# Alan-404/Conformer

Measured on AMD Instinct MI355X. Metric: encoder audio-frames/sec (B=32,T=1000,d=512,L=16), higher is better.
Workload: dtype f32

## Files before the change

### conformer_amd/_lib.py

```python
from __future__ import annotations

import ctypes
import os
from ctypes import c_char_p, c_float, c_int, c_int64, c_uint64, c_void_p

_HERE = os.path.dirname(os.path.abspath(__file__))
LIB_PATH = os.environ.get("CONFORMER_AMD_LIB") or os.path.join(_HERE, "lib", "libconformer_hip.so")

_P, _I, _L, _F, _U = c_void_p, c_int, c_int64, c_float, c_uint64
ABI_VERSION = 4

SIGNATURES = {
    "cfm_version": (c_int, []),
    "cfm_abi_version": (c_int, []),
    "cfm_gemm_bias_stats_f32": (c_int, [_P, _P, _P, _P, _P, _L, _I, _I, _L, _L, _P]),
    "cfm_gemm_bias_residual_stats_f32": (c_int, [_P, _P, _P, _P, _F, _P, _P, _L, _I, _I, _L, _L, _L, _P]),
    "cfm_gemm_splitk_f32": (c_int, [_I, _P, _P, _P, _P, _F, _P, _P, _I, _L, _I, _I, _L, _L, _L, _P]),
    "cfm_gemm_lnfold_f32": (c_int, [_I, _P, _P, _I, _F, _P, _P, _P, _P, _L, _I, _I, _L, _L, _P]),
    "cfm_layernorm_fwd_stats_f32": (c_int, [_P, _P, _P, _P, _P, _L, _I, _F, _P]),
    "cfm_ffn_pack_elems": (ctypes.c_int64, [_I, _I]),
    "cfm_ffn_pack_f32": (c_int, [_P, _P, _P, _I, _I, _P]),
    "cfm_rowgemm_pack_f32": (c_int, [_P, _P, _I, _I, _I, _P]),
    "cfm_rowchain_f32": (c_int, [_I, _I, _I, _I, _P, _L, _P, _P, _P, _L, _P, _L, _P, _I, _F, _P, _P, _P, _P, _F, _I, _P, _L, _P, _P, _P, _F,
                                 _P, _P, _P, _F, _P, _L, _L, _I, _P]),
# ... 33 lines not shown
    "cfm_subsample_conv1_bwd_d16_f32": (c_int, [_I, _P, _P, _P, _P, _P, _P, _I, _I, _I, _I, _P]),
    "cfm_reflect_pad_f32": (c_int, [_P, _P, _I, _L, _I, _L, _P]),
    "cfm_power_mel_log_f32": (c_int, [_P, _L, _P, _P, _I, _I, _I, _I, _F, _P]),
    "cfm_power_mel_log_mfma_f32": (c_int, [_P, _L, _P, _P, _I, _I, _I, _I, _I, _F, _P]),
    "cfm_dft_frames_f32": (c_int, [_P, _P, _P, _L, _I, _I, _I, _P]),
    "cfm_specaugment_apply_f32": (c_int, [_P, _I, _I, _I, _P, _I, _F, _P]),
    "cfm_gemm_bias_swish_save_f32": (c_int, [_P, _P, _P, _P, _P, _L, _I, _I, _L, _L, _P]),
    "cfm_gemm_bwd_f32": (c_int, [_P, _I, _L, _P, _I, _L, _P, _L, _F, _P, _L, _I, _I, _L, _I, _P]),
    "cfm_gemm_bwd_batched_f32": (c_int, [_P, _I, _L, _P, _I, _L, _P, _L, _F, _P, _L, _I, _I, _L, _I, _I, _I, _I,
                                         _L, _L, _L, _L, _L, _L, _F, _U, _P]),
    "cfm_gemm_train_f32": (c_int, [_I, _P, _P, _P, _P, _F, _P, _P, _L, _I, _I, _L, _L, _L, _F, _U, _P]),
    "cfm_relpos_attention_train_f32": (c_int, [_P, _P, _P, _L, _P, _L, _P, _P, _P, _P, _L, _P, _I, _I, _I, _I, _F, _U, _P]),
    "cfm_dropout_f32": (c_int, [_P, _P, _L, _F, _U, _P]),
    "cfm_dropout_out16_f32": (c_int, [_I, _P, _P, _L, _F, _U, _P]),
    "cfm_layernorm_bwd_dx_f32": (c_int, [_P, _P, _P, _P, _P, _P, _P, _L, _I, _P]),
    "cfm_layernorm_bwd_params_f32": (c_int, [_P, _P, _P, _P, _P, _P, _L, _I, _P]),
    "cfm_layernorm_bwd_f32": (c_int, [_P, _P, _P, _P, _P, _P, _P, _P, _P, _L, _I, _P, ctypes.c_size_t, _P]),
    "cfm_layernorm_bwd_workspace_bytes": (ctypes.c_size_t, [_L, _I]),
    "cfm_colsum_f32": (c_int, [_P, _L, _L, _I, _F, _P, _P]),
    "cfm_glu_fwd_f32": (c_int, [_P, _P, _L, _I, _P]),
    "cfm_glu_bwd_f32": (c_int, [_P, _P, _P, _L, _I, _P]),
    "cfm_dwconv_bn_swish_bwd_f32": (c_int, [_P, _P, _P, _P, _P, _P, _P, _P, _F, _I, _P, _P, _P, _P, _P, _P,
                                            _I, _I, _I, _I, _P]),
    "cfm_dwconv_bn_stats_workspace_bytes": (ctypes.c_size_t, [_I, _I, _I]),
    "cfm_dwconv_bn_stats_f32": (c_int, [_P, _P, _P, _P, _P, _P, _P, _F, _I, _I, _I, _I, _P, ctypes.c_size_t, _P]),
    "cfm_debug_attention_bwd_trace_f32": (c_int, [_P]),
    "cfm_debug_attention_bwd_trace_mfma16": (c_int, [_P]),
    "cfm_debug_gemm_mfma16_trace": (c_int, [_P]),
    "cfm_debug_gemm_mfma16_force_tile": (c_int, [_I]),
    "cfm_relpos_attention_bwd_mfma16_f32": (c_int, [_I, _P, _P, _P, _L, _P, _L, _P, _P, _P, _P, _P, _L, _P, _P, _P, _P, _L, _P, _L,
                                                    _P, _P, _I, _I, _I, _I, _F, _U, _P]),
    "cfm_relpos_attention_bwd_f32": (c_int, [_P, _P, _P, _L, _P, _L, _P, _P, _P, _P, _P, _L, _P, _P, _P, _P, _L, _P, _L, _P, _P,
                                             _I, _I, _I, _I, _F, _U, _I, _P]),
    "cfm_relu_bwd_f32": (c_int, [_P, _P, _P, _L, _P]),
    "cfm_subsample_conv2_bwd_weight_f32": (c_int, [_P, _P, _P, _I, _I, _I, _I, _P]),
    "cfm_pack_conv2_weight_t_f32": (c_int, [_P, _P, _I, _P]),
    "cfm_subsample_conv2_bwd_input_f32": (c_int, [_P, _P, _P, _I, _I, _I, _I, _P]),
    "cfm_subsample_conv1_bwd_f32": (c_int, [_P, _P, _P, _P, _P, _P, _I, _I, _I, _I, _P]),
    "cfm_adam_step_f32": (c_int, [_P, _I, _F, _F, _F, _F, _F, _F, _P]),
    "cfm_greedy_ctc_decode_f32": (c_int, [_P, _P, _P, _P, _P, _I, _I, _I, _I, _I, _P]),
    "cfm_ctc_beam_workspace_bytes": (ctypes.c_size_t, [_I, _I, _I, _I]),
    "cfm_ctc_beam_decode_f32": (c_int, [_P, _P, _I, _I, _I, _I, _I, _I, _F, _F, _I, _P, ctypes.c_size_t, _P, _P, _P, _P, _P]),
    "cfm_ngram_lm_pack_bytes": (ctypes.c_size_t, [_I, _P, _I, _L, _I, _L]),
    "cfm_ngram_lm_pack": (c_int, [_I, _P, _P, _P, _P, _I, _P, _P, _I, _I, _I, _I, _P, _P, _P, _P, ctypes.c_size_t]),
    "cfm_ngram_lm_score_f64": (c_int, [_P, _P, _P, _I, _I, _P, _P]),
    "cfm_ctc_beam_lm_workspace_bytes": (ctypes.c_size_t, [_I, _I, _I, _I]),
    "cfm_ctc_beam_lm_decode_f32": (c_int, [_P, _P, _I, _I, _I, _I, _I, _I, _F, _F, _I, _P, ctypes.c_double, ctypes.c_double,
                                           ctypes.c_double, _I, _P, ctypes.c_size_t, _P, _P, _P, _P, _P, _P]),
    "cfm_lstm_fwd_f32": (c_int, [_P, _P, _P, _P, _P, _P, _P, _I, _I, _I, _P]),
    "cfm_lstm_fwd_frag_f32": (c_int, [_P, _P, _P, _P, _P, _P, _P, _P, _I, _I, _I, _P]),
    "cfm_lstm_bwd_frag_f32": (c_int, [_P, _P, _P, _P, _P, _P, _P, _P, _I, _I, _I, _P]),
    "cfm_debug_lstm_trace": (c_int, [_P]),
    "cfm_debug_dw16_trace": (c_int, [_P]),
    "cfm_linear_bwd_weight_mfma16_f32": (c_int, [_I, _P, _I, _L, _P, _I, _L, _P, _L, _P, _I, _I, _L, _F, _P]),
    "cfm_lstm_fwd_mfma16_f32": (c_int, [_I, _P, _P, _P, _P, _P, _P, _P, _P, _I, _I, _I, _P]),
    "cfm_lstm_bwd_mfma16_f32": (c_int, [_I, _P, _P, _P, _P, _P, _P, _P, _P, _I, _I, _I, _P]),
    "cfm_lstm_bwd_f32": (c_int, [_P, _P, _P, _P, _P, _P, _P, _I, _I, _I, _P]),
    "cfm_swish_bn_eval_f32": (c_int, [_P, _P, _P, _P, _P, _F, _P, _L, _I, _P]),
    "cfm_swish_bn_stats_f32": (c_int, [_P, _P, _P, _P, _P, _F, _L, _I, _P]),
    "cfm_swish_bn_bwd_f32": (c_int, [_P, _P, _P, _P, _P, _F, _I, _P, _P, _P, _L, _I, _P]),
    "cfm_split_pack_elems": (ctypes.c_int64, [_I, _I, _I]),
    "cfm_split_pack_bf16_f32": (c_int, [_I, _P, _P, _I, _I, _P]),
    "cfm_gemm_split_bf16_f32": (c_int, [_I, _I, _P, _P, _P, _P, _F, _P, _L, _I, _I, _L, _L, _L, _P]),
    "cfm_subsample_conv2_relu_split_bf16_f32": (c_int, [_I, _P, _P, _P, _P, _I, _I, _I, _I, _P]),
    "cfm_ctc_workspace_floats": (ctypes.c_int64, [_I, _I, _I]),
    "cfm_ctc_loss_fwd_f32": (c_int, [_P, _P, _P, _L, _L, _P, _P, _I, _I, _I, _I, _I, _P, _P, _P]),
    "cfm_ctc_loss_bwd_f32": (c_int, [_P, _P, _P, _L, _L, _P, _P, _I, _I, _I, _I, _I, _P, _P, _P, _P]),
    "cfm_relpos_attention_rows_f32": (c_int, [_P, _P, _P, _L, _P, _L, _P, _P, _P, _P, _L, _I, _I, _I, _I, _I, _I, _I, _P, _P]),
    "cfm_debug_attention_trace_f32": (c_int, [_P, _P, _P, _L, _P, _L, _P, _P, _P, _P, _L, _I, _I, _I, _I, _P, _P]),
    "cfm_debug_set_bwd_tile": (c_int, [_I]),
    "cfm_debug_set_attention_waves": (c_int, [_I]),
    "cfm_debug_gemm_cfg_f32": (c_int, [_I, _P, _P, _P, _P, _F, _P, _L, _I, _I, _P, _P]),
    "cfm_debug_set_conv2_bk": (c_int, [_I]),
    "cfm_debug_ffn_trace": (c_int, [_P, _I]),
    "cfm_debug_ffn_variant": (c_int, [_I]),
    "cfm_debug_ffn_layout": (c_int, [_I, _I]),
    "cfm_relpos_table_f32": (c_int, [_P, _P, _I, _I, _P]),
    "cfm_relpos_attention_fwd_f32": (c_int, [_P, _P, _P, _L, _P, _L, _P, _P, _P, _P, _L, _P, _I, _I, _I, _I, _P]),
    "cfm_dwconv_bn_swish_fwd_f32": (c_int, [_P, _P, _P, _P, _P, _P, _P, _F, _P, _I, _I, _I, _I, _P]),
    "cfm_subsample_conv1_relu_f32": (c_int, [_P, _P, _P, _P, _I, _I, _I, _I, _P]),
    "cfm_pack_conv2_weight_f32": (c_int, [_P, _P, _I, _P]),
    "cfm_subsample_conv2_relu_f32": (c_int, [_P, _P, _P, _P, _I, _I, _I, _I, _P]),
    "cfm_pack_linear_weight_f32": (c_int, [_P, _P, _I, _I, _I, _P]),
}


class ConformerHipError(RuntimeError):
    pass


_lib = None


def load() -> ctypes.CDLL:
    global _lib
    if _lib is not None:
        return _lib
    if not os.path.exists(LIB_PATH):
        raise ConformerHipError(
            f"{LIB_PATH} is missing: build it with `python -m conformer_amd.build` "
            "(there is no CPU/eager fallback for the Conformer hot path)")
    import torch
    lib = ctypes.CDLL(LIB_PATH, mode=ctypes.RTLD_GLOBAL)
    try:
        lib.cfm_abi_version.restype = c_int
        got = int(lib.cfm_abi_version())
    except AttributeError:
        got = 0
    if got != ABI_VERSION:
        raise ConformerHipError(f"{LIB_PATH} implements C-ABI revision {got}, this binding needs {ABI_VERSION}: rebuild it with "
                                "`python -m conformer_amd.build`")
    for name, (res, args) in SIGNATURES.items():
        fn = getattr(lib, name)
        fn.restype = res
        fn.argtypes = args
    _lib = lib
    return lib


class CastItem(ctypes.Structure):
    _fields_ = [("src", ctypes.c_void_p), ("dst", ctypes.c_void_p), ("rows", ctypes.c_int64), ("cols", ctypes.c_int64),
                ("transpose", ctypes.c_int)]


CALLS = [0]


def check(status: int, what: str) -> None:
    CALLS[0] += 1
    if status != 0:
        msg = load().cfm_strerror(status).decode()
        raise ConformerHipError(f"{what} failed: {msg} (status {status})")
```

### conformer_amd/model/utils/convolution.py

```python
from typing import Optional, Tuple

import torch
import torch.nn as nn
import torch.nn.functional as F

from ... import autograd as ag
from ... import ops
from ._guard import PackCache, active_dropout, refuse_dropout
from .activation import GLU, Swish


class ConvolutionModule(nn.Module):
    def __init__(self, channels: int, kernel_size: int, dropout_rate: float = 0.0) -> None:
        super().__init__()
        self.layer_norm = nn.LayerNorm(normalized_shape=channels)
        self.pointwise_conv_1 = nn.Conv1d(channels, channels * 2, kernel_size=1)
        self.glu = GLU(dim=1)
        self.deepwise_conv = nn.Conv1d(channels, channels, kernel_size=kernel_size, padding=(kernel_size - 1) // 2,
                                       groups=channels)
        self.batch_norm = nn.BatchNorm1d(num_features=channels)
        self.swish = Swish()
        self.pointwise_conv_2 = nn.Conv1d(channels, channels, kernel_size=1)
        self.dropout = nn.Dropout(p=dropout_rate)
        self._packs = PackCache()

    def fused(self, x: torch.Tensor, residual: Optional[torch.Tensor] = None, stats: Optional[torch.Tensor] = None,
              emit_stats: bool = False):
        refuse_dropout(self, "ConvolutionModule")
        bn = self.batch_norm
        train_bn = bn.training or bn.running_mean is None
        if train_bn and (bn.momentum is None or not bn.track_running_stats):
            raise NotImplementedError("ConvolutionModule: only the default BatchNorm1d(momentum=0.1, "
                                      "track_running_stats=True) is built")
        if train_bn and not ag.needs_grad(self, x, residual):
            h = ops.layernorm(x, self.layer_norm.weight, self.layer_norm.bias, self.layer_norm.eps, for_gemm=True)
            g = ops.linear_glu(h, self.pointwise_conv_1.weight, self.pointwise_conv_1.bias)
            bm, bv = ops.dwconv_bn_batch_stats(g, self.deepwise_conv.weight, self.deepwise_conv.bias, bn.running_mean,
                                               bn.running_var, bn.momentum)
            bn.num_batches_tracked += 1
            s = ops.dwconv_bn_swish(g, self.deepwise_conv.weight, self.deepwise_conv.bias, bn.weight, bn.bias, bm, bv,
                                    bn.eps, for_gemm=True)
            if residual is None:
                return ops.linear(s, self.pointwise_conv_2.weight, self.pointwise_conv_2.bias)
            return ops.linear_residual(s, self.pointwise_conv_2.weight, self.pointwise_conv_2.bias, residual, 1.0)
        if ag.needs_grad(self, x, residual):
            if residual is not None and residual is not x:
                raise NotImplementedError("ConvolutionModule.fused: pass residual=x (block.py:23)")
            out = ag.ConvModuleFn.apply(x, self.layer_norm.weight, self.layer_norm.bias, self.pointwise_conv_1.weight,
                                        self.pointwise_conv_1.bias, self.deepwise_conv.weight, self.deepwise_conv.bias,
                                        bn.weight, bn.bias, bn.running_mean, bn.running_var,
                                        self.pointwise_conv_2.weight, self.pointwise_conv_2.bias,
                                        self.layer_norm.eps, bn.eps, train_bn, bn.momentum if train_bn else 0.0,
                                        active_dropout(self.dropout))
            if train_bn:
                bn.num_batches_tracked += 1
            return out if residual is not None else out - x
        if stats is not None:
            ln, pw1 = self.layer_norm, self.pointwise_conv_1
            wf, bf, cs = self._packs.get("ln_fold", (pw1.weight, pw1.bias, ln.weight, ln.bias),
                                         lambda: ops.fold_layernorm(pw1.weight, pw1.bias, ln.weight, ln.bias))
            g = ops.linear_lnfold(x, stats, wf, bf, cs, ln.eps, glu=True)
        else:
            h = ops.layernorm(x, self.layer_norm.weight, self.layer_norm.bias, self.layer_norm.eps, for_gemm=True)
            g = ops.linear_glu(h, self.pointwise_conv_1.weight, self.pointwise_conv_1.bias)
        s = ops.dwconv_bn_swish(g, self.deepwise_conv.weight, self.deepwise_conv.bias, bn.weight, bn.bias,
                                bn.running_mean, bn.running_var, bn.eps, for_gemm=True)
        if residual is None:
            if emit_stats:
                return ops.linear(s, self.pointwise_conv_2.weight, self.pointwise_conv_2.bias, emit_stats=True)
            return ops.linear(s, self.pointwise_conv_2.weight, self.pointwise_conv_2.bias)
        return ops.linear_residual(s, self.pointwise_conv_2.weight, self.pointwise_conv_2.bias, residual, 1.0, emit_stats=emit_stats)

    def forward(self, x: torch.Tensor) -> torch.Tensor:
        return self.fused(x)


class ConvolutionSubsampling(nn.Module):
    def __init__(self, channels: int) -> None:
        super().__init__()
        self.conv_1 = nn.Conv2d(1, channels, kernel_size=3, stride=2)
        self.act_1 = nn.ReLU()
        self.conv_2 = nn.Conv2d(channels, channels, kernel_size=3, stride=2)
        self.act_2 = nn.ReLU()
        self._packs = PackCache()

    @staticmethod
    def out_lengths(lengths: Optional[torch.Tensor]) -> Optional[torch.Tensor]:
        if lengths is None:
            return None
        if lengths.is_cuda and lengths.dtype == torch.int64:
            return ops.subsampled_lengths(lengths)
        return torch.div(torch.div(lengths - 1, 2, rounding_mode="floor") - 1, 2, rounding_mode="floor")

    def channel_last(self, x: torch.Tensor) -> torch.Tensor:
        if ag.needs_grad(self, x):
            if x.requires_grad:
                raise NotImplementedError("ConvolutionSubsampling: the gradient w.r.t. the input spectrogram is not "
                                          "built (the reference never needs it: the input is data)")
            return ag.SubsampleStemFn.apply(x, self.conv_1.weight, self.conv_1.bias, self.conv_2.weight, self.conv_2.bias)
        w2p = self._packs.get("w2p", (self.conv_2.weight,), lambda: ops.pack_conv2_weight(self.conv_2.weight))
        return ops.subsample_stem(x, self.conv_1.weight, self.conv_1.bias, w2p, self.conv_2.bias)

    def forward(self, x: torch.Tensor, lengths: Optional[torch.Tensor] = None) -> Tuple[torch.Tensor, Optional[torch.Tensor]]:
        h = self.channel_last(x)
        if h.dtype != torch.float32:
            h = h.float()
        B, T2, _ = h.shape
        C = self.conv_1.out_channels
        h = h.view(B, T2, -1, C).transpose(2, 3).reshape(B, T2, -1)
        return h, self.out_lengths(lengths)


class DepthWiseSeperableConvolution(nn.Module):

    def __init__(self, in_channels: int, out_channels: int) -> None:
        super().__init__()
        self.depth_wise_conv = nn.Conv2d(in_channels, out_channels, kernel_size=3, stride=2, groups=in_channels)
        self.point_wise_conv = nn.Conv2d(out_channels, out_channels, kernel_size=1)

    def forward(self, x: torch.Tensor):
        return self.point_wise_conv(self.depth_wise_conv(x))


class DownsamplingConvolution(nn.Module):

    def __init__(self, channels: int) -> None:
        super().__init__()
        self.conv_1 = DepthWiseSeperableConvolution(1, channels)
        self.conv_2 = DepthWiseSeperableConvolution(channels, channels)

    def forward(self, x: torch.Tensor, lengths: Optional[torch.Tensor]):
        h = F.relu(self.conv_2(F.relu(self.conv_1(x.unsqueeze(1)))))
        B, C, Fp, Tp = h.shape
        h = h.permute(0, 3, 1, 2).reshape(B, Tp, C * Fp)
        return h, ConvolutionSubsampling.out_lengths(lengths)
```

### conformer_amd/ops.py

```python
from __future__ import annotations

import threading
import ctypes
import weakref
from typing import Optional, Tuple

import torch

from . import _lib


def _stream() -> int:
    return torch.cuda.current_stream().cuda_stream


def _req(t: torch.Tensor, name: str, dtype=torch.float32) -> torch.Tensor:
    if not isinstance(t, torch.Tensor) or not t.is_cuda:
        raise _lib.ConformerHipError(
            f"{name}: expected a tensor on a HIP device, got {getattr(t, 'device', type(t))}; "
            "the Conformer hot path only exists as gfx950 kernels (no CPU fallback)")
    if t.dtype != dtype:
        raise _lib.ConformerHipError(f"{name}: expected dtype {dtype}, got {t.dtype}")
    return t if t.is_contiguous() else t.contiguous()

# ... 507 lines not shown
    if q16 or c16:
        esz = 2 if q16 else 4
        ctx = torch.empty(B, T, d, device=qkv.device, dtype=_DT16[prec] if c16 else torch.float32)
        st = _lib.load().cfm_relpos_attention_io16_mfma16_f32(prec, base, base + esz * d, base + 2 * esz * d, int(q16), d3,
                                                              pos.data_ptr(), ldp, u.data_ptr(), v.data_ptr(), _p(lengths),
                                                              ctx.data_ptr(), int(c16), d, B, T, n_heads, dh, _stream())
        _lib.check(st, "cfm_relpos_attention_io16_mfma16_f32")
        return ctx
    ctx = torch.empty(B, T, d, device=qkv.device, dtype=torch.float32)
    if prec:
        st = _lib.load().cfm_relpos_attention_mfma16_f32(prec, base, base + 4 * d, base + 8 * d, d3, pos.data_ptr(), ldp,
                                                         u.data_ptr(), v.data_ptr(), _p(lengths), ctx.data_ptr(), d, None,
                                                         B, T, n_heads, dh, 0.0, 0, _stream())
        _lib.check(st, "cfm_relpos_attention_mfma16_f32")
        return ctx
    st = _lib.load().cfm_relpos_attention_fwd_f32(base, base + 4 * d, base + 8 * d, d3, pos.data_ptr(), ldp,
                                                  u.data_ptr(), v.data_ptr(), _p(lengths), ctx.data_ptr(), d, None,
                                                  B, T, n_heads, dh, _stream())
    _lib.check(st, "cfm_relpos_attention_fwd_f32")
    return ctx


def relpos_attention_rows(qkv: torch.Tensor, pos: torch.Tensor, u: torch.Tensor, v: torch.Tensor, lengths: torch.Tensor,
                          n_heads: int, q_begin: int, q_count: int, ctx: torch.Tensor, keys_hint: Optional[int] = None
                          ) -> torch.Tensor:
    qkv = _req(qkv, "qkv"); u = _req(u, "content_bias"); v = _req(v, "position_bias"); ctx = _req(ctx, "ctx")
    B, T, d3 = qkv.shape
    d = d3 // 3
    if not (pos.is_cuda and pos.dtype == torch.float32 and pos.dim() == 2 and pos.stride(1) == 1 and pos.shape == (2 * T - 1, d)):
        raise _lib.ConformerHipError(f"pos: expected a ({2 * T - 1},{d}) fp32 HIP tensor with unit column stride")
    if ctx.shape != (B, T, d) or not qkv.is_contiguous() or not ctx.is_contiguous():
        raise _lib.ConformerHipError("relpos_attention_rows: qkv (B,T,3d) and ctx (B,T,d) must be contiguous cache buffers")
    lengths = _req(lengths, "lengths", torch.int64)
    prec = mfma16_prec()
    if prec != PREC_F32:
        base = qkv.data_ptr()
        st = _lib.load().cfm_relpos_attention_rows_mfma16_f32(prec, base, base + 4 * d, base + 8 * d, d3, pos.data_ptr(), pos.stride(0),
                                                              u.data_ptr(), v.data_ptr(), lengths.data_ptr(), ctx.data_ptr(), d, B, T,
                                                              n_heads, d // n_heads, int(q_begin), int(q_count), _stream())
        _lib.check(st, "cfm_relpos_attention_rows_mfma16_f32")
        return ctx
    tiles = ((T if keys_hint is None else min(int(keys_hint), T)) + 31) // 32
    blocks = B * n_heads * ((q_count + 127) // 128)
    nsplit = max(1, min(16, tiles // 8, -(-1024 // blocks)))
    ws = torch.empty(nsplit * B * q_count * (d + n_heads), device=qkv.device, dtype=torch.float32) if nsplit > 1 else None
    base = qkv.data_ptr()
    st = _lib.load().cfm_relpos_attention_rows_f32(base, base + 4 * d, base + 8 * d, d3, pos.data_ptr(), pos.stride(0),
                                                   u.data_ptr(), v.data_ptr(), lengths.data_ptr(), ctx.data_ptr(), d, B, T,
                                                   n_heads, d // n_heads, int(q_begin), int(q_count), nsplit, _p(ws), _stream())
    _lib.check(st, "cfm_relpos_attention_rows_f32")
    return ctx


def dwconv_bn_swish(g, w, b, bn_w, bn_b, bn_mean, bn_var, eps: float = 1e-5, for_gemm: bool = False) -> torch.Tensor:
    g = _req(g, "g"); w = _req(w, "dw weight"); b = _req(b, "dw bias")
    B, T, C = g.shape
    K = w.shape[-1]
    p16 = out16_ok(C) if for_gemm and K in (3, 7, 15, 31) else 0
    if p16:
        y = torch.empty(g.shape, device=g.device, dtype=_DT16[p16])
        st = _lib.load().cfm_dwconv_bn_swish_fwd_out16_f32(p16, g.data_ptr(), w.data_ptr(), b.data_ptr(), _req(bn_w, "bn_w").data_ptr(),
                                                           _req(bn_b, "bn_b").data_ptr(), _req(bn_mean, "bn_mean").data_ptr(),
                                                           _req(bn_var, "bn_var").data_ptr(), eps, y.data_ptr(), B, T, C, K,
                                                           _stream())
        _lib.check(st, "cfm_dwconv_bn_swish_fwd_out16_f32")
        return y
    y = _f32_like(g)
    st = _lib.load().cfm_dwconv_bn_swish_fwd_f32(g.data_ptr(), w.data_ptr(), b.data_ptr(), _req(bn_w, "bn_w").data_ptr(),
                                                 _req(bn_b, "bn_b").data_ptr(), _req(bn_mean, "bn_mean").data_ptr(),
                                                 _req(bn_var, "bn_var").data_ptr(), eps, y.data_ptr(), B, T, C, K,
                                                 _stream())
    _lib.check(st, "cfm_dwconv_bn_swish_fwd_f32")
    return y


def pack_conv2_weight(w2: torch.Tensor) -> torch.Tensor:
    w2 = _req(w2, "conv_2.weight")
    C = w2.shape[0]
    out = torch.empty(C, 9 * C, device=w2.device, dtype=torch.float32)
    _lib.check(_lib.load().cfm_pack_conv2_weight_f32(w2.data_ptr(), out.data_ptr(), C, _stream()), "cfm_pack_conv2_weight_f32")
    return out


def pack_linear_weight(wl: torch.Tensor, C: int, F2: int) -> torch.Tensor:
    wl = _req(wl, "linear.weight")
    out = _f32_like(wl)
    _lib.check(_lib.load().cfm_pack_linear_weight_f32(wl.data_ptr(), out.data_ptr(), wl.shape[0], C, F2, _stream()),
               "cfm_pack_linear_weight_f32")
    return out


def subsample_stem(x: torch.Tensor, w1, b1, w2p, b2) -> torch.Tensor:
    x = _req(x, "x"); w1 = _req(w1, "conv_1.weight"); b1 = _req(b1, "conv_1.bias")
    w2p = _req(w2p, "packed conv_2.weight"); b2 = _req(b2, "conv_2.bias")
    B, F, T = x.shape
    C = w1.shape[0]
    F1, T1 = (F - 1) // 2, (T - 1) // 2
    F2, T2 = (F1 - 1) // 2, (T1 - 1) // 2
    lib = _lib.load()
    p16 = out16_ok(C) if C % 64 == 0 else 0
    if p16:
        h1 = torch.empty(B, T1, F1, C, device=x.device, dtype=_DT16[p16])
        _lib.check(lib.cfm_subsample_conv1_relu_out16_f32(p16, x.data_ptr(), w1.data_ptr(), b1.data_ptr(), h1.data_ptr(), B, F,
                                                          T, C, _stream()), "cfm_subsample_conv1_relu_out16_f32")
        h2 = torch.empty(B, T2, F2 * C, device=x.device, dtype=_DT16[p16])
    else:
        h1 = torch.empty(B, T1, F1, C, device=x.device, dtype=torch.float32)
        _lib.check(lib.cfm_subsample_conv1_relu_f32(x.data_ptr(), w1.data_ptr(), b1.data_ptr(), h1.data_ptr(), B, F, T, C,
                                                    _stream()), "cfm_subsample_conv1_relu_f32")
        h2 = torch.empty(B, T2, F2 * C, device=x.device, dtype=torch.float32)
    _conv2_relu(lib, h1, w2p, b2, h2, B, F1, T1, C)
    return h2


def _conv2_relu(lib, h1, w2p, b2, h2, B, F1, T1, C):
    prec = mfma16_prec()
    if prec and C % 64 == 0:
        w16 = weight16(w2p, prec)
        _lib.check(lib.cfm_subsample_conv2_relu_mfma16_f32(prec, h1.data_ptr(), int(h1.dtype != torch.float32),
                                                           (w2p if w16 is None else w16).data_ptr(), int(w16 is not None),
                                                           b2.data_ptr(), h2.data_ptr(), int(h2.dtype != torch.float32), B, F1,
                                                           T1, C, _stream()), "cfm_subsample_conv2_relu_mfma16_f32")
    elif _fp32_planes and C % 64 == 0:
        ws = weight_split(w2p.view(C, 9 * C), _fp32_planes)
        _lib.check(lib.cfm_subsample_conv2_relu_split_bf16_f32(_fp32_planes, h1.data_ptr(), ws.data_ptr(), b2.data_ptr(),
                                                               h2.data_ptr(), B, F1, T1, C, _stream()),
                   "cfm_subsample_conv2_relu_split_bf16_f32")
    else:
        _lib.check(lib.cfm_subsample_conv2_relu_f32(h1.data_ptr(), w2p.data_ptr(), b2.data_ptr(), h2.data_ptr(), B, F1, T1,
                                                    C, _stream()), "cfm_subsample_conv2_relu_f32")


_ZERO_ARENA = {}
_ZERO_CHUNK = 16 << 20


def _zeros_split(device, dtype, *shapes):
    sizes = [int(torch.Size(sh).numel()) for sh in shapes]
    padded = [(n + 3) // 4 * 4 for n in sizes]
    total = sum(padded)
    if total >= _ZERO_CHUNK // 4 or torch.cuda.is_current_stream_capturing():
        buf, off = torch.zeros(total, device=device, dtype=dtype), 0
    else:
        key = (device, dtype, torch.cuda.current_stream(device).cuda_stream)
        ent = _ZERO_ARENA.get(key)
        if ent is None or ent[1] + total > ent[0].numel():
            ent = [torch.zeros(_ZERO_CHUNK, device=device, dtype=dtype), 0]
            _ZERO_ARENA[key] = ent
        buf, off = ent[0], ent[1]
        ent[1] = off + total
    outs = []
    for sh, n, pn in zip(shapes, sizes, padded):
        outs.append(buf[off:off + n].view(sh))
        off += pn
    return outs


def layernorm_train(x, weight, bias, eps: float = 1e-5, for_gemm: bool = False):
    x = _req(x, "x"); weight = _req(weight, "weight"); bias = _req(bias, "bias")
    d = x.shape[-1]
    rows = x.numel() // d
    mean = torch.empty(rows, device=x.device, dtype=torch.float32)
    rstd = torch.empty(rows, device=x.device, dtype=torch.float32)
    p16 = out16_ok(d) if for_gemm else 0
    if p16:
        y = torch.empty(x.shape, device=x.device, dtype=_DT16[p16])
        _lib.check(_lib.load().cfm_layernorm_fwd_out16_f32(p16, x.data_ptr(), weight.data_ptr(), bias.data_ptr(), y.data_ptr(),
                                                           mean.data_ptr(), rstd.data_ptr(), rows, d, eps, _stream()),
                   "cfm_layernorm_fwd_out16_f32")
        return y, mean, rstd
    y = _f32_like(x)
    st = _lib.load().cfm_layernorm_fwd_f32(x.data_ptr(), weight.data_ptr(), bias.data_ptr(), y.data_ptr(),
                                           mean.data_ptr(), rstd.data_ptr(), rows, d, eps, _stream())
    _lib.check(st, "cfm_layernorm_fwd_f32")
    return y, mean, rstd


def layernorm_bwd(x, weight, dy, mean, rstd, dres=None):
    x = _req(x, "x"); dy = _req(dy, "dy"); weight = _req(weight, "weight")
    d = x.shape[-1]
    rows = x.numel() // d
    lib = _lib.load()
    dx = _f32_like(x)
    if dres is not None:
        dres = _req(dres, "dres")
    dw, db = _zeros_split(x.device, x.dtype, (d,), (d,))
    if d <= 2048:
        nws = int(lib.cfm_layernorm_bwd_workspace_bytes(rows, d))
        ws = torch.empty(nws // 4, device=x.device, dtype=torch.float32)
        _lib.check(lib.cfm_layernorm_bwd_f32(x.data_ptr(), weight.data_ptr(), dy.data_ptr(), mean.data_ptr(), rstd.data_ptr(),
                                             _p(dres), dx.data_ptr(), dw.data_ptr(), db.data_ptr(), rows, d, ws.data_ptr(), nws,
                                             _stream()),
                   "cfm_layernorm_bwd_f32")
# ... 519 lines not shown
```

### include/conformer_hip.h

```cpp
#ifndef CONFORMER_HIP_H
#define CONFORMER_HIP_H

#include <stddef.h>
#include <stdint.h>

#ifdef __cplusplus
extern "C" {
#endif

typedef void* cfm_stream_t;

enum cfm_status {
    CFM_OK = 0,
    CFM_ERR_BAD_SHAPE = -1,
    CFM_ERR_UNSUPPORTED = -2,
    CFM_ERR_NULL = -3,
    CFM_ERR_LAUNCH = -4,
    CFM_ERR_DEVICE = -5,
    CFM_ERR_ALIGN = -6
};

int cfm_version(void);
int cfm_abi_version(void);
#define CFM_ABI_VERSION 4
const char* cfm_strerror(int status);
int cfm_device_check(void);

int cfm_layernorm_fwd_f32(const float* x, const float* gamma, const float* beta, float* y,
                          float* mean_or_null, float* rstd_or_null,
                          int64_t rows, int d, float eps, cfm_stream_t stream);

int cfm_gemm_bias_f32(const float* A, const float* W, const float* bias, float* C,
                      int64_t M, int N, int K, int64_t lda, int64_t ldc, cfm_stream_t stream);
int cfm_gemm_bias_swish_f32(const float* A, const float* W, const float* bias, float* C,
                            int64_t M, int N, int K, int64_t lda, int64_t ldc, cfm_stream_t stream);
int cfm_gemm_bias_relu_f32(const float* A, const float* W, const float* bias, float* C,
                           int64_t M, int N, int K, int64_t lda, int64_t ldc, cfm_stream_t stream);
int cfm_gemm_bias_glu_f32(const float* A, const float* W, const float* bias, float* C,
                          int64_t M, int n_out, int K, int64_t lda, int64_t ldc, cfm_stream_t stream);
int cfm_gemm_bias_residual_f32(const float* A, const float* W, const float* bias, const float* R,
                               float alpha, float* C, int64_t M, int N, int K,
                               int64_t lda, int64_t ldr, int64_t ldc, cfm_stream_t stream);

int cfm_gemm_splitk_f32(int epi, const float* A, const float* W, const float* bias, const float* R_or_null,
                        float alpha, float* C, float* workspace, int splits, int64_t M, int N, int K,
                        int64_t lda, int64_t ldr, int64_t ldc, cfm_stream_t stream);

int cfm_gemm_bias_stats_f32(const float* A, const float* W, const float* bias, float* C, float* stats_out,
                            int64_t M, int N, int K, int64_t lda, int64_t ldc, cfm_stream_t stream);
int cfm_gemm_bias_residual_stats_f32(const float* A, const float* W, const float* bias, const float* R,
                                     float alpha, float* C, float* stats_out, int64_t M, int N, int K,
                                     int64_t lda, int64_t ldr, int64_t ldc, cfm_stream_t stream);
int cfm_gemm_lnfold_f32(int epi, const float* A, const float* ln_stats, int ln_parts, float ln_eps,
                        const float* Wf, const float* bias_f, const float* colsum, float* C,
                        int64_t M, int N, int K, int64_t lda, int64_t ldc, cfm_stream_t stream);
int cfm_layernorm_fwd_stats_f32(const float* x, const float* gamma, const float* beta, float* y,
                                float* stats_out, int64_t rows, int d, float eps, cfm_stream_t stream);

int64_t cfm_ffn_pack_elems(int d, int hidden);
int cfm_ffn_pack_f32(const float* W1f, const float* W2, float* Wp, int d, int hidden, cfm_stream_t stream);
int cfm_ffn_fused_f32(const float* X, int64_t ldx, const float* ln_stats, int ln_parts, float ln_eps, const float* Wp,
                      const float* b1f, const float* colsum1, const float* b2, float alpha, float* Y, int64_t ldy,
                      int mode, float* stats_out, const float* gamma2, const float* beta2, float eps2, int64_t M,
                      int d, int hidden, cfm_stream_t stream);

int cfm_rowgemm_pack_f32(const float* W, float* Wp, int N, int d, int glu, cfm_stream_t stream);
int cfm_rowchain_f32(int pre, int core, int post, int mode, const float* X, int64_t ldx, const float* Wpre_packed,
                     const float* bpre, const float* R, int64_t ldr, float* Y1, int64_t ldy1, const float* ln_stats,
                     int ln_parts, float ln_eps, const float* Wffn_packed, const float* b1f, const float* colsum1,
                     const float* b2, float alpha, int hidden, float* Y, int64_t ldy, float* stats_out,
                     const float* gamma2, const float* beta2, float eps2, const float* Wpost_packed, const float* bpost,
                     const float* cspost, float post_eps, float* Z, int64_t ldz, int64_t M, int d, cfm_stream_t stream);
int64_t cfm_ffn_tile_stride_f4(int d);
int cfm_ffn_rotate(void);

int cfm_relpos_table_f32(const float* div_term, float* pe, int T, int d, cfm_stream_t stream);

int cfm_relpos_attention_fwd_f32(const float* q, const float* k, const float* v, int64_t ld,
                                 const float* pos, int64_t ldp, const float* u, const float* vbias,
                                 const int64_t* lengths_or_null, float* ctx, int64_t ldo,
                                 float* lse_or_null, int B, int T, int H, int dh, cfm_stream_t stream);

int cfm_dwconv_bn_swish_fwd_f32(const float* g, const float* w, const float* bias,
                                const float* bn_weight, const float* bn_bias,
                                const float* bn_mean, const float* bn_var, float bn_eps,
                                float* y, int B, int T, int C, int K, cfm_stream_t stream);

int cfm_subsample_conv1_relu_f32(const float* x, const float* w1, const float* b1, float* h1,
                                 int B, int F, int T, int C, cfm_stream_t stream);
int cfm_pack_conv2_weight_f32(const float* w2, float* w2p, int C, cfm_stream_t stream);
int cfm_subsample_conv2_relu_f32(const float* h1, const float* w2p, const float* b2, float* h2,
                                 int B, int F1, int T1, int C, cfm_stream_t stream);
int cfm_pack_linear_weight_f32(const float* wl, float* wlp, int d_out, int C, int F2, cfm_stream_t stream);

#define CFM_PREC_F32 0
#define CFM_PREC_BF16 1
#define CFM_PREC_FP16 2
int cfm_gemm_mfma16_f32(int prec, int epi, const void* A, int a_is_16bit, const void* W, int w_is_16bit,
                        const float* bias, const float* R_or_null, float alpha, void* C, int c_is_16bit,
                        void* Z_or_null, int z_is_16bit, int64_t M, int N, int K, int64_t lda, int64_t ldr,
                        int64_t ldc, float drop_p, uint64_t drop_seed, cfm_stream_t stream);
#define CFM_CAST_BATCH 48
typedef struct cfm_cast_item {
    const float* src;
    void* dst;
    int64_t rows, cols;
    int transpose;
} cfm_cast_item;
int cfm_cast16_multi_f32(int prec, const cfm_cast_item* items, int count, cfm_stream_t stream);
int cfm_layernorm_fwd_out16_f32(int prec, const float* x, const float* gamma, const float* beta, void* y16,
                                float* mean_or_null, float* rstd_or_null, int64_t rows, int d, float eps,
                                cfm_stream_t stream);
int cfm_cast16_f32(int prec, const float* src, void* dst, int64_t n, cfm_stream_t stream);
int cfm_relpos_attention_mfma16_f32(int prec, const float* q, const float* k, const float* v, int64_t ld,
                                    const float* pos, int64_t ldp, const float* u, const float* vbias,
                                    const int64_t* lengths_or_null, float* ctx, int64_t ldo, float* lse_or_null, int B,
                                    int T, int H, int dh, float drop_p, uint64_t drop_seed, cfm_stream_t stream);
int cfm_relpos_attention_rows_mfma16_f32(int prec, const float* q, const float* k, const float* v, int64_t ld,
                                         const float* pos, int64_t ldp, const float* u, const float* vbias,
                                         const int64_t* lengths, float* ctx, int64_t ldo, int B, int T, int H, int dh,
                                         int q_begin, int q_count, cfm_stream_t stream);
int cfm_relpos_attention_io16_mfma16_f32(int prec, const void* q, const void* k, const void* v, int qkv_is_16bit, int64_t ld,
                                         const float* pos, int64_t ldp, const float* u, const float* vbias,
                                         const int64_t* lengths_or_null, void* ctx, int ctx_is_16bit, int64_t ldo, int B, int T,
                                         int H, int dh, cfm_stream_t stream);
int cfm_subsample_conv2_relu_mfma16_f32(int prec, const void* h1, int h1_is_16bit, const void* w2p, int w_is_16bit,
                                        const float* b2, void* h2, int h2_is_16bit, int B, int F1, int T1, int C,
                                        cfm_stream_t stream);
int cfm_subsample_conv1_relu_out16_f32(int prec, const float* x, const float* w1, const float* b1, void* h1, int B, int F,
                                       int T, int C, cfm_stream_t stream);
int cfm_gemm_bwd_batched_mfma16_f32(int prec, const float* A, int a_col, int64_t lda, const void* B, int b_col,
                                    int b_is_16bit, int64_t ldb, const void* Z_or_null, int z_is_16bit, int64_t ldz, float alpha, void* C,
                                    int64_t ldc, int c_is_16bit, int I, int J, int64_t Kc, int allow_split, int accumulate,
                                    int nbatch, int nb1, int64_t sa0, int64_t sa1, int64_t sb0, int64_t sb1,
                                    int64_t sc0, int64_t sc1, float drop_p, uint64_t drop_seed,
                                    int operands_zero_padded4, cfm_stream_t stream);
int cfm_linear_bwd_weight_mfma16_f32(int prec, const void* dy, int dy_is_16bit, int64_t ldy, const void* x,
                                     int x_is_16bit, int64_t ldx, float* dw, int64_t ldw, float* db_or_null, int N,
                                     int K, int64_t M, float alpha, cfm_stream_t stream);
int64_t cfm_subsample_conv2_rowtab_elems(int B, int F1, int T1);
int cfm_subsample_conv2_bwd_weight_h16_mfma16_f32(int prec, const void* dz2, int dz2_is_16bit, const void* h1_16,
                                                  int* rowtab_scratch, float* dw2p, float* db2_or_null, int B, int F1, int T1,
                                                  int C, cfm_stream_t stream);
int cfm_dwconv_bn_swish_fwd_out16_f32(int prec, const float* g, const float* w, const float* bias, const float* bn_weight,
                                      const float* bn_bias, const float* bn_mean, const float* bn_var, float bn_eps,
                                      void* y16, int B, int T, int C, int K, cfm_stream_t stream);
int cfm_glu_bwd_out16_f32(int prec, const float* z, const float* dy, void* dz16, int64_t rows, int n, cfm_stream_t stream);
int cfm_relu_bwd_out16_f32(int prec, const float* y, const float* dy, void* dz16, int64_t n, cfm_stream_t stream);
int cfm_subsample_conv2_bwd_input_fwdkernel_mfma16_f32(int prec, const void* dz2, int dz2_is_16bit, const void* w2c16,
                                                       const float* zero_bias, float* dh1, int B, int F1, int T1,
                                                       int C, cfm_stream_t stream);
int cfm_subsample_conv2_bwd_input_fwdkernel_out16_mfma16_f32(int prec, const void* dz2, int dz2_is_16bit, const void* w2c16,
                                                             const float* zero_bias, void* dh1_16, int B, int F1, int T1, int C,
                                                             cfm_stream_t stream);
int cfm_subsample_conv1_bwd_d16_f32(int prec, const float* x, const float* w1, const float* b1, const void* dh1_16, float* dw1,
                                    float* db1, int B, int F, int T, int C, cfm_stream_t stream);
int cfm_subsample_conv2_bwd_weight_mfma16_f32(int prec, const float* dz2, const float* h1, float* dw2p, int B, int F1,
                                              int T1, int C, cfm_stream_t stream);
int cfm_subsample_conv2_bwd_input_mfma16_f32(int prec, const float* dz2, const float* w2c, float* dh1, int B, int F1,
                                             int T1, int C, cfm_stream_t stream);

int cfm_reflect_pad_f32(const float* x, float* xp, int B, int64_t L, int pad, int64_t ld_out, cfm_stream_t stream);
int cfm_power_mel_log_f32(const float* spec, int64_t ld_spec, const float* fb, float* out, int B, int T,
                          int n_bins, int n_mels, float floor_value, cfm_stream_t stream);
int cfm_power_mel_log_mfma_f32(const float* spec, int64_t ld_spec, const float* fbT, float* out, int B, int T,
                               int rows_per_utt, int n_bins, int n_mels, float floor_value, cfm_stream_t stream);
int cfm_dft_frames_f32(const float* wave, const float* basis, float* spec, int64_t rows, int n_cols, int n_fft,
                       int hop, cfm_stream_t stream);
int cfm_specaugment_apply_f32(float* spec, int B, int F, int T, const int* bands, int nbands, float value,
                              cfm_stream_t stream);


int cfm_gemm_bias_swish_save_f32(const float* A, const float* W, const float* bias, float* C, float* Z,
                                 int64_t M, int N, int K, int64_t lda, int64_t ldc, cfm_stream_t stream);

int cfm_gemm_bwd_f32(const float* A, int a_col, int64_t lda, const float* B, int b_col, int64_t ldb,
// ... 181 lines not shown
```

Before: 1.598 million.

## Add Winograd-style strided conv2 path for the subsampling stem

Adds a Winograd-like decomposition of the stride-2 3x3 subsampling conv2. Each 2x2 output block is computed from nine partial-product planes, using input differences and pre-summed weight taps, by an MFMA GEMM kernel. A combine kernel then adds the planes, applies bias and ReLU. This cuts the multiply count of the stem convolution but adds a large intermediate planes buffer that costs extra memory traffic and a second launch. It is enabled by default when C is a multiple of 256 and the fp32 path is active.

```diff
diff --git a/conformer_amd/_lib.py b/conformer_amd/_lib.py
--- a/conformer_amd/_lib.py
+++ b/conformer_amd/_lib.py
@@ -139,6 +139,9 @@
     "cfm_pack_conv2_weight_f32": (c_int, [_P, _P, _I, _P]),
     "cfm_subsample_conv2_relu_f32": (c_int, [_P, _P, _P, _P, _I, _I, _I, _I, _P]),
     "cfm_pack_linear_weight_f32": (c_int, [_P, _P, _I, _I, _I, _P]),
+    "cfm_conv2_wino_plane_elems": (c_int64, [_I, _I, _I, _I]),
+    "cfm_pack_conv2_wino_weight_f32": (c_int, [_P, _P, _I, _P]),
+    "cfm_subsample_conv2_wino_relu_f32": (c_int, [_P, _P, _P, _P, _P, _I, _I, _I, _I, _P]),
 }
 
 
diff --git a/conformer_amd/csrc/conv2_wino_f32.hip b/conformer_amd/csrc/conv2_wino_f32.hip
--- /dev/null
+++ b/conformer_amd/csrc/conv2_wino_f32.hip
@@ -0,0 +1,304 @@
+#include <algorithm>
+#include <utility>
+
+#include "gemm_shared.h"
+
+namespace {
+
+#define WINO_MFMA_SLICE(FA, FB)                                                                             \
+    _Pragma("unroll") for (int e = 0; e < 4; ++e)                                                           \
+    _Pragma("unroll") for (int mt = 0; mt < TM; ++mt)                                                       \
+    _Pragma("unroll") for (int nt = 0; nt < TN; ++nt)                                                       \
+        acc[mt][nt] = __builtin_amdgcn_mfma_f32_32x32x2f32(FB[nt][e], FA[mt][e], acc[mt][nt], 0, 0, 0)
+
+template <typename Fn, int... I>
+__device__ __forceinline__ void static_for_seq(Fn& f, std::integer_sequence<int, I...>) {
+    (f(std::integral_constant<int, I>{}), ...);
+}
+template <int N, typename Fn>
+__device__ __forceinline__ void static_for(Fn&& f) {
+    static_for_seq(f, std::make_integer_sequence<int, N>{});
+}
+
+__host__ __device__ constexpr int wino_nt(int a) { return a == 1 ? 1 : 2; }
+__host__ __device__ constexpr int wino_terms(int p) { return wino_nt(p / 3) * wino_nt(p % 3); }
+
+struct WinoArgs {
+    const float* h1; const float* w; float* planes;
+    int64_t M;
+    unsigned h1_bytes;
+    int T1, F1, C, TI, TJ;
+    unsigned tiles_m, tiles_n;
+    unsigned grp_blk[4];
+};
+
+
+template <int ST, int SF>
+__device__ __forceinline__ void wino_tile(const WinoArgs& g, int p, int64_t m0, int n0, float* lds) {
+    constexpr int BM = 256, BN = 256, WN = 4, TM = 4, TN = 2, BK = 16, LDSR = BK + 4, NT = ST * SF, SPC = 2 * NT;
+    constexpr int NPX = (ST == 2 ? 2 : 1) * (SF == 2 ? 2 : 1);
+    float* As = lds;
+    float* Bs = lds + 2 * BM * LDSR;
+    const int a = p / 3, b = p - 3 * (p / 3);
+    const int sg_t = a >> 1, sg_f = b >> 1;
+
+    const int tid = threadIdx.x, lane = tid & 63;
+    const int wave = __builtin_amdgcn_readfirstlane(tid >> 6);
+    const int wr = wave / WN, wc = wave % WN;
+    const int li = lane & 31, hf = lane >> 5;
+
+    constexpr int CPR = BK / 4, RPP = 512 / CPR, PA = BM / RPP, PB = BN / RPP;
+    const int chunk = tid & (CPR - 1), srow = tid / CPR;
+    unsigned row_off[PA];
+    const int64_t pos_per_b = (int64_t)g.TI * g.TJ;
+#pragma unroll
+    for (int i = 0; i < PA; ++i) {
+        int64_t m = m0 + srow + RPP * i;
+        if (m >= g.M) m = g.M - 1;
+        const int64_t bb = m / pos_per_b;
+        const int r = (int)(m - bb * pos_per_b);
+        const int ib = r / g.TJ, jb = r - ib * g.TJ;
+        row_off[i] = (unsigned)((((bb * g.T1 + 4 * ib) * g.F1 + 4 * jb) * (int64_t)g.C + chunk * 4) * 4);
+    }
+    const __amdgpu_buffer_rsrc_t h1_rsrc = __builtin_amdgcn_make_buffer_rsrc(const_cast<float*>(g.h1), (short)0, (int)g.h1_bytes, 0x00020000);
+    const unsigned pix_t[3] = {(unsigned)((ST == 2 ? 4 * sg_t : 2) * g.F1 * g.C * 4), (unsigned)(2 * g.F1 * g.C * 4),
+                               (unsigned)((1 + 2 * sg_t) * g.F1 * g.C * 4)};
+    const unsigned pix_f[3] = {(unsigned)((SF == 2 ? 4 * sg_f : 2) * g.C * 4), (unsigned)(2 * g.C * 4), (unsigned)((1 + 2 * sg_f) * g.C * 4)};
+    int64_t woff = 0;
+    for (int q = 0; q < p; ++q) woff += wino_terms(q);
+    const int K = NT * g.C;
+    const __amdgpu_buffer_rsrc_t w_rsrc = __builtin_amdgcn_make_buffer_rsrc(const_cast<float*>(g.w + woff * g.C * g.C), (short)0,
+                                                                            K * g.C * 4, 0x00020000);
+    unsigned w_off[PB];
+#pragma unroll
+    for (int i = 0; i < PB; ++i) w_off[i] = (unsigned)(((n0 + srow + RPP * i) * K + chunk * 4) * 4);
+
+    f32x4 raw[PA][NPX], rb[PB];
+    auto load_tile = [&](auto U_, int c32, int half) __attribute__((always_inline)) {
+        constexpr int U = decltype(U_)::value, UT = U / SF, UF = U % SF;
+        constexpr int NXT = (ST == 2 && UT == 0) ? 2 : 1, NYF = (SF == 2 && UF == 0) ? 2 : 1;
+        constexpr int X1 = ST == 2 ? (UT == 0 ? 0 : 2) : 0, Y1 = SF == 2 ? (UF == 0 ? 0 : 2) : 0;
+        const unsigned ci4 = (unsigned)(32 * c32 + 16 * half) * 4;
+#pragma unroll
+        for (int x = 0; x < NXT; ++x)
+#pragma unroll
+            for (int y = 0; y < NYF; ++y) {
+                const unsigned po = pix_t[X1 + x] + pix_f[Y1 + y] + ci4;
+#pragma unroll
+                for (int i = 0; i < PA; ++i)
+                    raw[i][x * NYF + y] = __builtin_bit_cast(f32x4, __builtin_amdgcn_raw_buffer_load_b128(h1_rsrc, row_off[i] + po, 0, 0));
+            }
+        const unsigned k4 = (unsigned)(NT * 32 * c32 + 32 * U + 16 * half) * 4;
+#pragma unroll
+        for (int i = 0; i < PB; ++i) rb[i] = __builtin_bit_cast(f32x4, __builtin_amdgcn_raw_buffer_load_b128(w_rsrc, w_off[i] + k4, 0, 0));
+    };
+    auto store_tile = [&](auto U_, int buf) __attribute__((always_inline)) {
+        constexpr int U = decltype(U_)::value, UT = U / SF, UF = U % SF;
+        constexpr int NXT = (ST == 2 && UT == 0) ? 2 : 1, NYF = (SF == 2 && UF == 0) ? 2 : 1;
+#pragma unroll
+        for (int i = 0; i < PA; ++i) {
+            const f32x4* px = raw[i];
+            f32x4 v;
+            if constexpr (NXT == 2 && NYF == 2) v = (px[0] - px[1]) - (px[2] - px[3]);
+            else if constexpr (NXT * NYF == 2) v = px[0] - px[1];
+            else v = px[0];
+            *reinterpret_cast<f32x4*>(As + (buf * BM + srow + RPP * i) * LDSR + chunk * 4) = v;
+        }
+#pragma unroll
+        for (int i = 0; i < PB; ++i)
+            *reinterpret_cast<f32x4*>(Bs + (buf * BN + srow + RPP * i) * LDSR + chunk * 4) = rb[i];
+    };
+
+    f32x16 acc[TM][TN];
+#pragma unroll
+    for (int i = 0; i < TM; ++i)
+#pragma unroll
+        for (int j = 0; j < TN; ++j)
+#pragma unroll
+            for (int r = 0; r < 16; ++r) acc[i][j][r] = 0.f;
+
+    const int a_row = wr * (BM / 2) + li, b_row = wc * (BN / WN) + li;
+    f32x4 fa0[TM], fb0[TN], fa1[TM], fb1[TN];
+    auto read_frags = [&](f32x4 (&fa)[TM], f32x4 (&fb)[TN], int buf, int c) __attribute__((always_inline)) {
+#pragma unroll
+        for (int t = 0; t < TM; ++t)
+            fa[t] = *reinterpret_cast<const f32x4*>(As + (buf * BM + a_row + 32 * t) * LDSR + 8 * c + 4 * hf);
+#pragma unroll
+        for (int t = 0; t < TN; ++t)
+            fb[t] = *reinterpret_cast<const f32x4*>(Bs + (buf * BN + b_row + 32 * t) * LDSR + 8 * c + 4 * hf);
+    };
+
+    const int nch = g.C / 32;
+    load_tile(std::integral_constant<int, 0>{}, 0, 0);
+    store_tile(std::integral_constant<int, 0>{}, 0);
+    load_tile(std::integral_constant<int, 0>{}, 0, 1);
+    __syncthreads();
+    read_frags(fa0, fb0, 0, 0);
+    for (int c32 = 0; c32 < nch; ++c32) {
+        static_for<SPC>([&](auto S_) __attribute__((always_inline)) {
+            constexpr int S = decltype(S_)::value;
+            constexpr int S1 = (S + 1) % SPC, S2 = (S + 2) % SPC;
+            const int cur = S & 1;
+            const bool more = S + 1 < SPC || c32 + 1 < nch;
+            read_frags(fa1, fb1, cur, 1);
+            __builtin_amdgcn_sched_barrier(0);
+            WINO_MFMA_SLICE(fa0, fb0);
+            __builtin_amdgcn_sched_barrier(0);
+            if (more) store_tile(std::integral_constant<int, S1 / 2>{}, cur ^ 1);
+            load_tile(std::integral_constant<int, S2 / 2>{}, S + 2 < SPC ? c32 : min(c32 + 1, nch - 1), S2 & 1);
+            __syncthreads();
+            if (more) read_frags(fa0, fb0, cur ^ 1, 0);
+            __builtin_amdgcn_sched_barrier(0);
+            WINO_MFMA_SLICE(fa1, fb1);
+            __builtin_amdgcn_sched_barrier(0);
+        });
+    }
+
+    __syncthreads();
+    GemmArgs ge{};
+    ge.C = g.planes + (int64_t)p * g.M * g.C;
+    ge.M = g.M; ge.N = g.C; ge.K = K; ge.ldc = g.C; ge.alpha = 1.f;
+    gemm_epilogue_rows<BM, BN, EPI_BIAS, TM, TN, 2, false, EPF_INFER | EPF_NO_BIAS, WN>(ge, acc, m0, n0, wr, wc, lane,
+                                                                                        lds + wave * 32 * (32 * TN + 4));
+}
+
+__global__ __launch_bounds__(512, 2) void conv2_wino_gemm_kernel(const WinoArgs g) {
+    constexpr int LDS_STAGE = 2 * (256 + 256) * 20;
+    static_assert(8 * 32 * (32 * 2 + 4) <= LDS_STAGE, "the row-major epilogue scratch must fit the staging buffers");
+    __shared__ __attribute__((aligned(16))) float lds[LDS_STAGE];
+    const unsigned bid = blockIdx.x;
+    const int grp = bid < g.grp_blk[1] ? 0 : (bid < g.grp_blk[2] ? 1 : 2);
+    const unsigned npat = grp == 2 ? 1u : 4u;
+    const unsigned ntile = npat * g.tiles_m * g.tiles_n;
+    const unsigned local = bid - g.grp_blk[grp], per_xcd = (g.grp_blk[grp + 1] - g.grp_blk[grp]) / 8;
+    const unsigned tile = (local & 7u) * per_xcd + (local >> 3);
+    if (tile >= ntile) return;
+    const unsigned tn = tile % g.tiles_n, rest = tile / g.tiles_n;
+    const unsigned pi = rest % npat, tm = rest / npat;
+    const int p = (int)(((grp == 0 ? 0x8620u : grp == 1 ? 0x5371u : 0x4u) >> (4 * pi)) & 15u);
+    const int64_t m0 = (int64_t)tm * 256;
+    const int n0 = (int)tn * 256;
+    const int nta = wino_nt(p / 3), ntb = wino_nt(p % 3);
+    if (nta == 2 && ntb == 2) wino_tile<2, 2>(g, p, m0, n0, lds);
+    else if (nta == 2) wino_tile<2, 1>(g, p, m0, n0, lds);
+    else if (ntb == 2) wino_tile<1, 2>(g, p, m0, n0, lds);
+    else wino_tile<1, 1>(g, p, m0, n0, lds);
+}
+
+__global__ __launch_bounds__(256) void conv2_wino_combine_kernel(const float* __restrict__ planes, const float* __restrict__ b2,
+                                                                 float* __restrict__ h2, int64_t M, int T2, int F2, int TI,
+                                                                 int TJ, int C) {
+    const int c4n = C / 4;
+    const int64_t idx = (int64_t)blockIdx.x * blockDim.x + threadIdx.x;
+    if (idx >= M * c4n) return;
+    const int64_t m = idx / c4n;
+    const int c = (int)(idx - m * c4n) * 4;
+    const int64_t per_b = (int64_t)TI * TJ;
+    const int64_t bb = m / per_b;
+    const int r = (int)(m - bb * per_b);
+    const int ib = r / TJ, jb = r - ib * TJ;
+    const int64_t plane = M * (int64_t)C;
+    f32x4 P[9];
+#pragma unroll
+    for (int q = 0; q < 9; ++q) P[q] = __builtin_nontemporal_load(reinterpret_cast<const f32x4*>(planes + q * plane + m * C + c));
+    const f32x4 bias = *reinterpret_cast<const f32x4*>(b2 + c);
+#pragma unroll
+    for (int rt = 0; rt < 2; ++rt) {
+        const int t2 = 2 * ib + rt;
+        if (t2 >= T2) continue;
+        const f32x4 u0 = P[3 * rt + 0] + P[3 * rt + 1], u1 = P[3 * rt + 1] + P[3 * rt + 2];
+        const f32x4 v0 = P[3 * rt + 3] + P[3 * rt + 4], v1 = P[3 * rt + 4] + P[3 * rt + 5];
+#pragma unroll
+        for (int s = 0; s < 2; ++s) {
+            const int f2 = 2 * jb + s;
+            if (f2 >= F2) continue;
+            const f32x4 y = (s == 0 ? u0 + v0 : u1 + v1) + bias;
+            f32x4 o;
+#pragma unroll
+            for (int e = 0; e < 4; ++e) o[e] = fmaxf(y[e], 0.f);
+            *reinterpret_cast<f32x4*>(h2 + (((bb * T2 + t2) * F2) + f2) * (int64_t)C + c) = o;
+        }
+    }
+}
+
+__global__ __launch_bounds__(256) void pack_conv2_wino_kernel(const float* __restrict__ w2, float* __restrict__ wp, int C) {
+    const int p = blockIdx.y, nt = wino_terms(p);
+    const int64_t idx = (int64_t)blockIdx.x * blockDim.x + threadIdx.x;
+    const int64_t K = (int64_t)nt * C;
+    if (idx >= K * C) return;
+    const int64_t co = idx / K;
+    const int k = (int)(idx - co * K);
+    const int c32 = k / (32 * nt), rem = k - c32 * 32 * nt, u = rem / 32, ci = 32 * c32 + (rem & 31);
+    int64_t off = 0;
+    for (int q = 0; q < p; ++q) off += wino_terms(q);
+    const int a = p / 3, b = p % 3, sfn = wino_nt(b);
+    const int ut = u / sfn, uf = u % sfn;
+    auto taps = [](int pat, int term, int (&tp)[2]) {
+        if (pat == 1) { tp[0] = 0; tp[1] = 2; return 2; }
+        tp[0] = term == 0 ? 2 * (pat >> 1) : 1;
+        return 1;
+    };
+    int tt[2], tf[2];
+    const int ntt = taps(a, ut, tt), ntf = taps(b, uf, tf);
+    double s = 0.0;
+    const float* wc = w2 + (co * C + ci) * 9;
+    for (int x = 0; x < ntt; ++x)
+        for (int y = 0; y < ntf; ++y) s += (double)wc[tf[y] * 3 + tt[x]];
+    wp[off * C * C + idx] = (float)s;
+}
+
+}
+
+extern "C" int64_t cfm_conv2_wino_plane_elems(int B, int F1, int T1, int C) {
+    if (B <= 0 || F1 < 3 || T1 < 3 || C <= 0) return 0;
+    const int64_t TI = ((T1 - 1) / 2 + 1) / 2, TJ = ((F1 - 1) / 2 + 1) / 2;
+    return 9 * (int64_t)B * TI * TJ * C;
+}
+
+extern "C" int cfm_pack_conv2_wino_weight_f32(const float* w2, float* wp, int C, cfm_stream_t stream) {
+    CFM_REQUIRE(w2 && wp, CFM_ERR_NULL);
+    CFM_REQUIRE(C > 0 && C % 32 == 0, CFM_ERR_BAD_SHAPE);
+    const int64_t most = 4 * (int64_t)C * C;
+    hipLaunchKernelGGL(pack_conv2_wino_kernel, dim3((unsigned)((most + 255) / 256), 9), dim3(256), 0,
+                       static_cast<hipStream_t>(stream), w2, wp, C);
+    return cfm_launch_status();
+}
+
+extern "C" int cfm_subsample_conv2_wino_relu_f32(const float* h1, const float* wp, const float* b2, float* planes, float* h2,
+                                                 int B, int F1, int T1, int C, cfm_stream_t stream) {
+    CFM_REQUIRE(h1 && wp && b2 && planes && h2, CFM_ERR_NULL);
+    CFM_REQUIRE(B > 0 && F1 >= 3 && T1 >= 3, CFM_ERR_BAD_SHAPE);
+    CFM_REQUIRE(C > 0 && C % 256 == 0, CFM_ERR_UNSUPPORTED);
+    CFM_REQUIRE(CFM_ALIGNED16(h1) && CFM_ALIGNED16(wp) && CFM_ALIGNED16(b2) && CFM_ALIGNED16(planes) && CFM_ALIGNED16(h2),
+                CFM_ERR_ALIGN);
+    const int64_t utt_bytes = (int64_t)T1 * F1 * C * 4, limit = (1LL << 32) - (1LL << 26);
+    CFM_REQUIRE(utt_bytes <= limit && 5LL * F1 * C * 4 < (1LL << 26), CFM_ERR_UNSUPPORTED);
+    const int T2 = (T1 - 1) / 2, F2 = (F1 - 1) / 2;
+    WinoArgs g{};
+    g.w = wp;
+    g.T1 = T1; g.F1 = F1; g.C = C; g.TI = (T2 + 1) / 2; g.TJ = (F2 + 1) / 2;
+    g.tiles_n = (unsigned)(C / 256);
+    const int64_t per_b = (int64_t)g.TI * g.TJ;
+    const int group = (int)std::min<int64_t>(B, limit / utt_bytes);
+    hipStream_t s = static_cast<hipStream_t>(stream);
+    for (int b0 = 0; b0 < B; b0 += group) {
+        const int nb = std::min(group, B - b0);
+        g.h1 = h1 + b0 * (utt_bytes / 4);
+        g.h1_bytes = (unsigned)(nb * utt_bytes);
+        g.M = nb * per_b;
+        g.planes = planes + 9 * (b0 * per_b) * C;
+        g.tiles_m = (unsigned)((g.M + 255) / 256);
+        const unsigned group_n[3] = {4, 4, 1};
+        g.grp_blk[0] = 0;
+        for (int q = 0; q < 3; ++q) g.grp_blk[q + 1] = g.grp_blk[q] + (group_n[q] * g.tiles_m * g.tiles_n + 7) / 8 * 8;
+        hipLaunchKernelGGL(conv2_wino_gemm_kernel, dim3(g.grp_blk[3]), dim3(512), 0, s, g);
+        int st = cfm_launch_status();
+        if (st) return st;
+        const int64_t threads = g.M * (C / 4);
+        hipLaunchKernelGGL(conv2_wino_combine_kernel, dim3((unsigned)((threads + 255) / 256)), dim3(256), 0, s, g.planes, b2,
+                           h2 + (int64_t)b0 * T2 * F2 * C, g.M, T2, F2, g.TI, g.TJ, C);
+        st = cfm_launch_status();
+        if (st) return st;
+    }
+    return 0;
+}
diff --git a/conformer_amd/model/utils/convolution.py b/conformer_amd/model/utils/convolution.py
--- a/conformer_amd/model/utils/convolution.py
+++ b/conformer_amd/model/utils/convolution.py
@@ -99,7 +99,10 @@
                                           "built (the reference never needs it: the input is data)")
             return ag.SubsampleStemFn.apply(x, self.conv_1.weight, self.conv_1.bias, self.conv_2.weight, self.conv_2.bias)
         w2p = self._packs.get("w2p", (self.conv_2.weight,), lambda: ops.pack_conv2_weight(self.conv_2.weight))
-        return ops.subsample_stem(x, self.conv_1.weight, self.conv_1.bias, w2p, self.conv_2.bias)
+        w2w = None
+        if ops.conv2_winograd_ok(self.conv_2.weight.shape[0]):
+            w2w = self._packs.get("w2w", (self.conv_2.weight,), lambda: ops.pack_conv2_wino_weight(self.conv_2.weight))
+        return ops.subsample_stem(x, self.conv_1.weight, self.conv_1.bias, w2p, self.conv_2.bias, w2w=w2w)
 
     def forward(self, x: torch.Tensor, lengths: Optional[torch.Tensor] = None) -> Tuple[torch.Tensor, Optional[torch.Tensor]]:
         h = self.channel_last(x)
diff --git a/conformer_amd/ops.py b/conformer_amd/ops.py
--- a/conformer_amd/ops.py
+++ b/conformer_amd/ops.py
@@ -613,6 +613,28 @@
     return out
 
 
+_CONV2_WINOGRAD = __import__("os").environ.get("CONFORMER_AMD_CONV2_WINOGRAD", "1") == "1"
+
+
+def set_conv2_winograd(on: bool) -> bool:
+    global _CONV2_WINOGRAD
+    prev, _CONV2_WINOGRAD = _CONV2_WINOGRAD, bool(on)
+    return prev
+
+
+def conv2_winograd_ok(C: int) -> bool:
+    return bool(_CONV2_WINOGRAD and C % 256 == 0 and not mfma16_prec() and not _fp32_planes)
+
+
+def pack_conv2_wino_weight(w2: torch.Tensor) -> torch.Tensor:
+    w2 = _req(w2, "conv_2.weight")
+    C = w2.shape[0]
+    out = torch.empty(25 * C * C, device=w2.device, dtype=torch.float32)
+    _lib.check(_lib.load().cfm_pack_conv2_wino_weight_f32(w2.data_ptr(), out.data_ptr(), C, _stream()),
+               "cfm_pack_conv2_wino_weight_f32")
+    return out
+
+
 def pack_linear_weight(wl: torch.Tensor, C: int, F2: int) -> torch.Tensor:
     wl = _req(wl, "linear.weight")
     out = _f32_like(wl)
@@ -621,7 +643,7 @@
     return out
 
 
-def subsample_stem(x: torch.Tensor, w1, b1, w2p, b2) -> torch.Tensor:
+def subsample_stem(x: torch.Tensor, w1, b1, w2p, b2, w2w=None) -> torch.Tensor:
     x = _req(x, "x"); w1 = _req(w1, "conv_1.weight"); b1 = _req(b1, "conv_1.bias")
     w2p = _req(w2p, "packed conv_2.weight"); b2 = _req(b2, "conv_2.bias")
     B, F, T = x.shape
@@ -640,6 +662,12 @@
         _lib.check(lib.cfm_subsample_conv1_relu_f32(x.data_ptr(), w1.data_ptr(), b1.data_ptr(), h1.data_ptr(), B, F, T, C,
                                                     _stream()), "cfm_subsample_conv1_relu_f32")
         h2 = torch.empty(B, T2, F2 * C, device=x.device, dtype=torch.float32)
+        if w2w is not None and conv2_winograd_ok(C):
+            planes = torch.empty(int(lib.cfm_conv2_wino_plane_elems(B, F1, T1, C)), device=x.device, dtype=torch.float32)
+            _lib.check(lib.cfm_subsample_conv2_wino_relu_f32(h1.data_ptr(), _req(w2w, "Winograd conv_2.weight").data_ptr(),
+                                                             b2.data_ptr(), planes.data_ptr(), h2.data_ptr(), B, F1, T1, C,
+                                                             _stream()), "cfm_subsample_conv2_wino_relu_f32")
+            return h2
     _conv2_relu(lib, h1, w2p, b2, h2, B, F1, T1, C)
     return h2
 
diff --git a/include/conformer_hip.h b/include/conformer_hip.h
--- a/include/conformer_hip.h
+++ b/include/conformer_hip.h
@@ -92,6 +92,10 @@
 int cfm_subsample_conv2_relu_f32(const float* h1, const float* w2p, const float* b2, float* h2,
                                  int B, int F1, int T1, int C, cfm_stream_t stream);
 int cfm_pack_linear_weight_f32(const float* wl, float* wlp, int d_out, int C, int F2, cfm_stream_t stream);
+int64_t cfm_conv2_wino_plane_elems(int B, int F1, int T1, int C);
+int cfm_pack_conv2_wino_weight_f32(const float* w2, float* wwp, int C, cfm_stream_t stream);
+int cfm_subsample_conv2_wino_relu_f32(const float* h1, const float* wwp, const float* b2, float* planes, float* h2,
+                                      int B, int F1, int T1, int C, cfm_stream_t stream);
 
 #define CFM_PREC_F32 0
 #define CFM_PREC_BF16 1
```

Measured after the change: 1.664 million (median of 6 runs). 4.1% higher.
